# THUDM/CogView

Measured on AMD Instinct MI355X. Metric: train tokens/sec/node (seq1089, 4B GPT) at 1/2/4/8 MI355X; % MFMA roofline, higher is better.
Workload: dtype fp16

## Files before the change

### cogview_amd/_lib.py

```python
import ctypes as C
import os

_HERE = os.path.dirname(os.path.abspath(__file__))
LIB_PATH = os.environ.get("COGVIEW_HIP_LIB") or os.path.join(_HERE, "lib", "libcogview_hip.so")

F16, BF16, F32 = 0, 1, 2
EPI_BIAS, EPI_GELU, EPI_DGELU, EPI_DROPOUT, EPI_ABSMAX, EPI_ACCUM, EPI_COLSUM = 1, 2, 4, 8, 16, 32, 64
EPI_GELU_DAUX, EPI_MULAUX = 128, 256

_ERR = {1: "bad argument (shape / alignment / dtype)", 2: "kernel launch failure", 3: "unsupported combination"}


class CogviewHipError(RuntimeError):
    pass


class GemmDesc(C.Structure):
    _fields_ = [
        ("dtype", C.c_int), ("trans_a", C.c_int), ("trans_b", C.c_int),
        ("M", C.c_int), ("N", C.c_int), ("K", C.c_int),
        ("A", C.c_void_p), ("lda", C.c_int),
        ("B", C.c_void_p), ("ldb", C.c_int),
        ("C", C.c_void_p), ("ldc", C.c_int),
        ("out_f32", C.c_int), ("flags", C.c_int),
# ... 148 lines not shown


CONV_4X4_S2, CONV_1X1, CONVT_4X4_S2, CONV_3X3_S1 = 0, 1, 2, 3
CONV_FP32, CONV_BF16X3 = 0, 1

_vp, _i, _f, _u64, _i64, _sz = C.c_void_p, C.c_int, C.c_float, C.c_uint64, C.c_int64, C.c_size_t

SIGNATURES = {
    "cogv_version": (_i, []),
    "cogv_arch": (C.c_char_p, []),
    "cogv_gemm": (_i, [C.POINTER(GemmDesc), _vp]),
    "cogv_gemm_workspace_bytes": (_sz, [C.POINTER(GemmDesc)]),
    "cogv_gemm_pick_splitk": (_i, [_i, _i, _i]),
    "cogv_gemm_grouped": (_i, [C.POINTER(GemmDesc), _i, _vp]),
    "cogv_gemm_colsum_rows": (_i, [_i]),
    "cogv_colsum_finalize": (_i, [_i, _vp, _i, _i, _vp, _i, _vp]),
    "cogv_gemm_pick_splitk_tiles": (_i, [_i, _i]),
    "cogv_sandwich_ln_fwd": (_i, [_i, _vp, _vp, _vp, _vp, _vp, _vp, _vp, _vp, _vp, _i, _i, _f, _i, _vp]),
    "cogv_sandwich_ln_bwd": (_i, [_i, _vp, _vp, _vp, _vp, _vp, _vp, _vp, _vp, _vp, _vp, _i, _i, _i, _f, _u64, _u64,
                                  _vp, _sz, _i, _vp]),
    "cogv_sandwich_ln_bwd_marked": (_i, [_i, _vp, _vp, _vp, _vp, _vp, _vp, _vp, _vp, _vp, _vp, _i, _i, _i, _f, _vp, _sz, _i, _vp]),
    "cogv_ln_bwd_workspace_bytes": (_sz, [_i, _i]),
    "cogv_sandwich_ln_bwd_pair": (_i, [_i, _vp, _vp, _vp, _vp, _vp, _vp, _vp, _vp, _vp, _vp, _vp, _vp, _vp, _vp, _vp, _vp, _vp, _i, _i, _i, _f,
                                       _vp, _sz, _vp]),
    "cogv_ln_bwd_pair_workspace_bytes": (_sz, [_i, _i]),
    "cogv_ln_bwd_num_blocks": (_i, [_i]),
    "cogv_ln_bwd_plan": (_i, [_i, _i, _i, _f, _i, _i, C.POINTER(C.c_int)]),
    "cogv_ln_bwd_pair_plan": (_i, [_i, _i, _f, C.POINTER(C.c_int)]),
    "cogv_gemm_reserve_cus": (_i, [_i]),
    "cogv_gemm_plan": (_i, [C.POINTER(GemmDesc), _i, _i, C.POINTER(C.c_int)]),
    "cogv_attention_fwd": (_i, [C.POINTER(AttnDesc), _vp]),
    "cogv_attention_bwd": (_i, [C.POINTER(AttnDesc), _vp]),
    "cogv_attention_plan": (_i, [C.POINTER(AttnDesc), _i, C.POINTER(C.c_int)]),
    "cogv_gemv_ln": (_i, [C.POINTER(GemmDesc), C.POINTER(LnPrologue), _vp]),
    "cogv_gemv_attn": (_i, [C.POINTER(GemmDesc), _vp, _i, _i, _vp]),
    "cogv_attention_decode": (_i, [C.POINTER(AttnDecodeDesc), _vp]),
    "cogv_attention_decode_chunk": (_i, [C.POINTER(AttnDecodeChunkDesc), _vp]),
    "cogv_quantize_rows_e4m3": (_i, [_i, _vp, _i, _i, _i, _vp, _i, _vp, _vp]),
    "cogv_gemm_w8": (_i, [C.POINTER(GemmDesc), C.POINTER(W8Weight), _vp]),
    "cogv_gemv_ln_w8": (_i, [C.POINTER(GemmDesc), C.POINTER(LnPrologue), C.POINTER(W8Weight), _vp]),
    "cogv_gemv_attn_w8": (_i, [C.POINTER(GemmDesc), C.POINTER(W8Weight), _vp, _i, _i, _vp]),
    "cogv_gemv_plan": (_i, [_i, C.POINTER(GemmDesc), C.POINTER(W8Weight), _i, C.POINTER(C.c_int)]),
    "cogv_quantize_rows_mxfp4": (_i, [_i, _vp, _i, _i, _i, _vp, _i, _vp, _i, _vp]),
    "cogv_gemm_w4": (_i, [C.POINTER(GemmDesc), C.POINTER(W4Weight), _vp]),
    "cogv_gemv_ln_w4": (_i, [C.POINTER(GemmDesc), C.POINTER(LnPrologue), C.POINTER(W4Weight), _vp]),
    "cogv_gemv_attn_w4": (_i, [C.POINTER(GemmDesc), C.POINTER(W4Weight), _vp, _i, _i, _vp]),
    "cogv_gemv_w4_plan": (_i, [_i, C.POINTER(GemmDesc), C.POINTER(W4Weight), _i, C.POINTER(C.c_int)]),
    "cogv_gemm_rows": (_i, [C.POINTER(GemmDesc), _vp]),
    "cogv_gemm_rows_plan": (_i, [C.POINTER(GemmDesc), C.POINTER(C.c_int)]),
    "cogv_kv_quantize_e4m3": (_i, [_i, _vp, _i64, _i64, _i, _i, _i, _vp, _i64, _vp, _i64, _i, _i, _vp]),
    "cogv_attention_decode_kv8": (_i, [C.POINTER(AttnDecodeKv8Desc), _vp]),
    "cogv_attention_decode_workspace_bytes": (_sz, [_i, _i, _i]),
    "cogv_attention_keep_bits_bytes": (_sz, [_i, _i, _i, _i]),
    "cogv_sparse_slot_reduce": (_i, [_i, _vp, _vp, _vp, _vp, _vp, _i64, _i, _i64, _i, _i, _i, _i, _i, _i, _i, _vp]),
    "cogv_embedding_fwd": (_i, [_i, _vp, _vp, _i64, _i64, _vp, _vp, _vp, _i64, _vp, _vp, _i64, _i, _f, _u64, _u64, _i, _vp]),
    "cogv_embedding_bwd": (_i, [_i, _vp, _vp, _vp, _i64, _i64, _vp, _vp, _i64, _vp, _i64, _i, _f, _u64, _u64, _vp, _sz, _i, _vp]),
    "cogv_embedding_bwd_workspace_bytes": (_sz, [_i64, _i64]),
    "cogv_gelu_fwd": (_i, [_i, _vp, _vp, _sz, _vp]),
    "cogv_gelu_bwd": (_i, [_i, _vp, _vp, _vp, _sz, _vp]),
    "cogv_dropout": (_i, [_i, _vp, _vp, _sz, _f, _u64, _u64, _vp, _vp]),
    "cogv_add": (_i, [_i, _vp, _vp, _vp, _sz, _vp, _vp]),
    "cogv_add_stream": (_i, [_i, _vp, _vp, _vp, _sz, _vp, _vp]),
    "cogv_scale": (_i, [_i, _vp, _vp, _sz, _f, _vp]),
    "cogv_absmax": (_i, [_i, _vp, _sz, _vp, _vp]),
    "cogv_colsum": (_i, [_i, _vp, _i, _i, _i, _vp, _i, _vp, _sz, _vp]),
    "cogv_colsum_workspace_bytes": (_sz, [_i, _i]),
# ... 156 lines not shown
```

### cogview_amd/csrc/attention.hip

```cpp
#include "common.cuh"
#include "cogview_hip.h"

#include <type_traits>

namespace {

constexpr int HD = 64;
constexpr int NT = 256;
constexpr float MASKED = -10000.0f;
constexpr int TILE = 8192;
#ifndef COGV_ATTN_STAGES
#define COGV_ATTN_STAGES 2
#endif
constexpr int NSTG = COGV_ATTN_STAGES;
static_assert(NSTG == 2 || NSTG == 3, "ring of two or three stages");
constexpr int COLSUM_SMEM = (128 * 68 + 256) * 4;

constexpr int DMA_TILE = 2;
template <int SIZE_, int DMAS_, bool COLSUM_> struct RingStage {
  static constexpr int SIZE = SIZE_, DMAS = DMAS_, INDEX = NSTG * SIZE_;
  static constexpr int dynamic_lds(int index_slots) {
    return ((COLSUM_ && INDEX < COLSUM_SMEM) ? COLSUM_SMEM : INDEX) + ((index_slots * 4 + 15) / 16) * 16;
  }
};
struct FwdStage : RingStage<2 * TILE, 2 * DMA_TILE, false> { static constexpr int K = 0, V = TILE; };
constexpr int DQ_KW_PITCH = 256;
template <bool KB> struct DqStage : RingStage<2 * TILE + (KB ? 4 * DQ_KW_PITCH : 0), 2 * DMA_TILE + (KB ? 1 : 0), true> {
  static constexpr int K = 0, V = TILE, KW = 2 * TILE, KW_PITCH = DQ_KW_PITCH;
};
constexpr int DKDV_KW_PITCH = 272;
template <bool KB> struct DkdvStage : RingStage<2 * TILE + 512 + (KB ? 4 * DKDV_KW_PITCH : 256), 2 * DMA_TILE + 3, true> {
  static constexpr int Q = 0, DO = TILE, LSE = 2 * TILE, D = LSE + 256;
  static constexpr int RK = D + 256, KW = D + 256, KW_PITCH = DKDV_KW_PITCH;
};

struct AttnArgs {
  const void* q; const void* k; const void* v; void* o;
  const void* dout; void* dq; void* dk; void* dv;
  float* lse; float* dvec;
  float* colsum_ws;
  uint32_t* keepbits;
  const void* mask; long long mask_bs;
  const int* kv_index; long long kv_index_bs;
  long long kv_index_gs; int sp_w, sp_npiv; float sp_bias;
  long long q_bs, k_bs, v_bs, o_bs, do_bs, dq_bs, dk_bs, dv_bs;
  int q_rs, k_rs, v_rs, o_rs, do_rs, dq_rs, dk_rs, dv_rs;
  int B, H, s_q, s_k, sep_k;
  float scale;
  uint32_t thr16; float keep_scale; uint32_t rng_key;
};

struct BlockId { int bx, head, z; bool ok; };
__device__ __forceinline__ BlockId xcd_block_id(int nx, int H, int Z, bool heavy_last) {
  const int L = blockIdx.x, x = L & 7, j = L >> 3;
  const int ul = j / nx, k = j - ul * nx;
  const int u = ul * 8 + x;
  BlockId id;
  id.ok = u < H * Z;
  id.z = u / H; id.head = u - id.z * H;
  id.bx = heavy_last ? nx - 1 - k : k;
  return id;
}

typedef __attribute__((address_space(3))) void lds_void_t;
typedef __attribute__((address_space(1))) const void gbl_void_t;

template <int N> __device__ __forceinline__ void wait_vmcnt() { asm volatile("s_waitcnt vmcnt(%0)" ::"n"(N) : "memory"); }

__device__ __forceinline__ int aswz(int row) { return (((row >> 1) & 1) << 2) | ((row >> 2) & 3); }

template <typename T>
__device__ __forceinline__ void dma_tile(const T* base, long long rs, int row0, int nrows, char* lds, int wave, int lane,
                                         const int* lds_index = nullptr) {
#pragma unroll
  for (int i = 0; i < DMA_TILE; ++i) {
    const int piece = wave + 4 * i;
    const int row = piece * 8 + (lane >> 3);
    const int c = (lane & 7) ^ aswz(row);
    int gr = min(row0 + row, nrows - 1);
    if (lds_index) {
      const uint32_t a = (uint32_t)(uintptr_t)(lds_index + gr);
      asm volatile("ds_read_b32 %0, %1\n\ts_waitcnt lgkmcnt(0)" : "=v"(gr) : "v"(a) : "memory");
// ... 87 lines not shown
__device__ __forceinline__ bool keep_of(const u32x2& r, int i, uint32_t thr16) {
  return (i & 1) ? (r[i >> 1] >= (thr16 << 16)) : ((r[i >> 1] & 0xffffu) >= thr16);
}

template <typename T, int SB>
__device__ __forceinline__ void tr_frags_issue(uint32_t tile_addr, const uint32_t (&loff)[2], TrRaw (&r)[2][2]) {
#pragma unroll
  for (int d = 0; d < 2; ++d) { tr_issue<SB * 32>(tile_addr, loff[d], r[0][d]); tr_issue<SB * 32 + 16>(tile_addr, loff[d], r[1][d]); }
}

template <typename T, int SB>
__device__ __forceinline__ void tr_frags_sync(uint32_t tile_addr, const uint32_t (&loff)[2], TrRaw (&r)[2][2]) {
  constexpr int S0 = SB * 32, S1 = SB * 32 + 16;
  constexpr int XA = (((S0 >> 3) & 1) << 1) << 4, XB = ((((S0 + 8) >> 3) & 1) << 1) << 4;
  constexpr int XC = (((S1 >> 3) & 1) << 1) << 4, XD = ((((S1 + 8) >> 3) & 1) << 1) << 4;
  uint32_t a[2][4];
#pragma unroll
  for (int d = 0; d < 2; ++d) {
    a[d][0] = tile_addr + S0 * 128 + (loff[d] ^ XA);
    a[d][1] = tile_addr + (S0 + 8) * 128 + (loff[d] ^ XB);
    a[d][2] = tile_addr + S1 * 128 + (loff[d] ^ XC);
    a[d][3] = tile_addr + (S1 + 8) * 128 + (loff[d] ^ XD);
  }
  asm volatile(
      "ds_read_b64_tr_b16 %0, %8\n\tds_read_b64_tr_b16 %1, %9\n\tds_read_b64_tr_b16 %2, %10\n\tds_read_b64_tr_b16 %3, %11\n\t"
      "ds_read_b64_tr_b16 %4, %12\n\tds_read_b64_tr_b16 %5, %13\n\tds_read_b64_tr_b16 %6, %14\n\tds_read_b64_tr_b16 %7, %15\n\t"
      "s_waitcnt lgkmcnt(0)"
      : "=&v"(r[0][0].lo), "=&v"(r[0][0].hi), "=&v"(r[1][0].lo), "=&v"(r[1][0].hi),
        "=&v"(r[0][1].lo), "=&v"(r[0][1].hi), "=&v"(r[1][1].lo), "=&v"(r[1][1].hi)
      : "v"(a[0][0]), "v"(a[0][1]), "v"(a[0][2]), "v"(a[0][3]), "v"(a[1][0]), "v"(a[1][1]), "v"(a[1][2]), "v"(a[1][3])
      : "memory");
}

__device__ __forceinline__ void tile_colsum(const float (&vals)[2][16], float* lds, float* dst, int lane, int wave) {
  constexpr int PITCH = 68;
  const int fr = lane & 31, fg = lane >> 5;
  float* row = lds + (wave * 32 + fr) * PITCH;
#pragma unroll
  for (int d = 0; d < 2; ++d)
#pragma unroll
    for (int gq = 0; gq < 4; ++gq)
      *reinterpret_cast<f32x4*>(row + 32 * d + 8 * gq + 4 * fg) =
          f32x4{vals[d][4 * gq], vals[d][4 * gq + 1], vals[d][4 * gq + 2], vals[d][4 * gq + 3]};
  __syncthreads();
  const int col = threadIdx.x & 63, slice = threadIdx.x >> 6;
  float s0 = 0.f, s1 = 0.f;
#pragma unroll
  for (int r = 0; r < 32; r += 2) {
    s0 += lds[(slice * 32 + r) * PITCH + col];
    s1 += lds[(slice * 32 + r + 1) * PITCH + col];
  }
  float* red = lds + 128 * PITCH;
  red[slice * 64 + col] = s0 + s1;
  __syncthreads();
  if (threadIdx.x < 64) dst[threadIdx.x] = red[threadIdx.x] + red[64 + threadIdx.x] + red[128 + threadIdx.x] + red[192 + threadIdx.x];
  __syncthreads();
}

template <bool IDX> __device__ __forceinline__ int* stage_index_table(const AttnArgs& p, int b, int gblk, char* behind_ring) {
  if (!(IDX && p.kv_index)) return nullptr;
  int* lidx = reinterpret_cast<int*>(behind_ring);
  const int* gi = p.kv_index + (long long)b * p.kv_index_bs + (long long)gblk * p.kv_index_gs;
  for (int i = threadIdx.x; i < p.s_k; i += NT) lidx[i] = gi[i];
  __syncthreads();
  return lidx;
}
struct SlotAttrs { unsigned long long masked, pivot; };
__device__ __forceinline__ SlotAttrs slot_attrs(const int* lidx, int kb, int lane, const AttnArgs& p) {
  int raw;
  const uint32_t ia = (uint32_t)(uintptr_t)(lidx + min(kb * 64 + lane, p.s_k - 1));
  asm volatile("ds_read_b32 %0, %1\n\ts_waitcnt lgkmcnt(0)" : "=v"(raw) : "v"(ia) : "memory");
  SlotAttrs a;
  a.masked = __ballot(raw < 0); a.pivot = __ballot(kb * 64 + lane < p.sp_npiv);
  return a;
}
__device__ __forceinline__ void apply_slot_attrs(f32x16& s, const SlotAttrs& a, int sb, int fg, float masked_raw, float bias_raw) {
  const uint32_t fm = (uint32_t)(a.masked >> (32 * sb)) >> (4 * fg), pm = (uint32_t)(a.pivot >> (32 * sb)) >> (4 * fg);
#pragma unroll
  for (int e = 0; e < 16; ++e) {
    const int bit = elem_idx(e);
    float v = s[e];
    v = ((fm >> bit) & 1u) ? masked_raw : v;
    v += ((pm >> bit) & 1u) ? bias_raw : 0.f;
    s[e] = v;
  }
}
template <typename T> __device__ __forceinline__ void apply_mask_tensor(f32x16& s, float (&mk)[16], const AttnArgs& p, int b, int myq,
                                                                        int kfirst, int fg, float masked_raw) {
  const T* mrow = reinterpret_cast<const T*>(p.mask) + (long long)b * p.mask_bs + (long long)min(myq, p.s_q - 1) * p.s_k;
#pragma unroll
  for (int e = 0; e < 16; ++e) {
    const int key = kfirst + 4 * fg + elem_idx(e);
    mk[e] = HT<T>::to_f(mrow[min(key, p.s_k - 1)]);
    s[e] = fmaf(s[e], mk[e], masked_raw * (1.f - mk[e]));
  }
}
template <int NF> __device__ __forceinline__ void mask_edge(f32x16* s, int kfirst, int q0w, int myq, int off, int fg, const AttnArgs& p,
                                                            float masked_raw) {
  const bool all_visible = (kfirst + (32 * NF - 1) <= q0w + off) || (kfirst + (32 * NF - 1) < p.sep_k);
  if (!all_visible || kfirst + 32 * NF > p.s_k) {
#pragma unroll
    for (int sb = 0; sb < NF; ++sb) {
      const int base = kfirst + sb * 32 + 4 * fg;
      mask_frag(s[sb], myq + off - base, p.sep_k - base, p.s_k - base, masked_raw);
    }
  }
}

template <typename T, bool IDX, int DROP>
__global__ __launch_bounds__(NT, 2) void attn_fwd_kernel(const AttnArgs p) {
  const bool drop = DROP < 0 ? (p.thr16 != 0u) : (DROP != 0);
  extern __shared__ __attribute__((aligned(16))) char smem[];
  using L = FwdStage;
  const int lane = threadIdx.x & 63;
  const int wave = __builtin_amdgcn_readfirstlane(threadIdx.x >> 6);
  const int fr = lane & 31, fg = lane >> 5;
  const int nblk_x = (p.s_q + 127) >> 7;
  const BlockId bid = xcd_block_id(nblk_x, p.H, p.B, true);
  if (!bid.ok) return;
  const int b = bid.z, head = bid.head;
  const int q0 = bid.bx * 128, q0w = q0 + wave * 32;
  const bool spw = IDX && p.sp_w > 0;
  const int gblk = spw ? q0 / p.sp_w : 0;
  const int off = spw ? (p.s_k - p.sp_w - gblk * p.sp_w) : (p.s_k - p.s_q);
  const T* Q = reinterpret_cast<const T*>(p.q) + b * p.q_bs + head * HD;
  const T* K = reinterpret_cast<const T*>(p.k) + b * p.k_bs + head * HD;
  const T* V = reinterpret_cast<const T*>(p.v) + b * p.v_bs + head * HD;
  const int myq = q0w + fr;
  const bool wave_active = q0w < p.s_q;

  typename HT<T>::v8 qf[4];
#pragma unroll
  for (int t = 0; t < 4; ++t) qf[t] = load_frag_global<T>(Q + (long long)myq * p.q_rs + 16 * t + 8 * fg, myq < p.s_q);

  const int q_last = min(p.s_q, q0 + 128) - 1;
  const int kend_blk = min(p.s_k, max(q_last + off + 1, p.sep_k));
  const int nkb = (kend_blk + 63) >> 6;
  const int qw_last = min(p.s_q, q0w + 32) - 1;
  const int kend_w = wave_active ? min(p.s_k, max(qw_last + off + 1, p.sep_k)) : 0;

  f32x16 oacc[2];
#pragma unroll
  for (int d = 0; d < 2; ++d)
#pragma unroll
    for (int e = 0; e < 16; ++e) oacc[d][e] = 0.f;
  float m_run = -INFINITY, l_run = 0.f;
  const float sl2 = p.scale * 1.4426950408889634f;
  const float masked_raw = MASKED / p.scale;
  const long long arow = ((long long)b * p.H + head) * p.s_q + myq;
  const RowKey cb = row_key(p.rng_key, (unsigned long long)arow);
  const float kofs = drop ? __builtin_amdgcn_logf(p.keep_scale) : 0.f;
  const uint32_t loff[2] = {tr_lane_off(0, lane) ^ tr_lane_fix(lane), tr_lane_off(1, lane) ^ tr_lane_fix(lane)};
  const uint32_t smem_addr = (uint32_t)(uintptr_t)smem;

  int* const lidx = stage_index_table<IDX>(p, b, gblk, smem + L::INDEX);
  const float sp_bias_raw = spw ? p.sp_bias / p.scale : 0.f;
  auto issue = [&](int kb, int st) {
    dma_tile<T>(K, p.k_rs, kb * 64, p.s_k, smem + st * L::SIZE + L::K, wave, lane, lidx);
    dma_tile<T>(V, p.v_rs, kb * 64, p.s_k, smem + st * L::SIZE + L::V, wave, lane, lidx);
  };
  static_assert(L::DMAS == 2 * DMA_TILE, "issue(): K tile, V tile");
  uint32_t* const kwp = DROP == 2 ? p.keepbits + ((((long long)b * p.H + head) * ((p.s_k + 63) >> 6)) * 2 + fg) * p.s_q + min(myq, p.s_q - 1) : nullptr;
  if (nkb > 0) { issue(0, 0); if (NSTG > 2) issue(nkb > 1 ? 1 : 0, 1); }
  int st = 0;
  for (int kb = 0; kb < nkb; ++kb) {
    wait_vmcnt<(NSTG - 2) * L::DMAS>();
    __builtin_amdgcn_s_barrier();
    issue(min(kb + NSTG - 1, nkb - 1), st == 0 ? NSTG - 1 : st - 1);
    if (kb * 64 < kend_w) {
      const char* lk = smem + st * L::SIZE + L::K;
      const uint32_t lv = smem_addr + st * L::SIZE + L::V;
      f32x16 sacc[2];
#pragma unroll
      for (int sb = 0; sb < 2; ++sb) {
#pragma unroll
        for (int e = 0; e < 16; ++e) sacc[sb][e] = 0.f;
#pragma unroll
        for (int t = 0; t < 4; ++t)
          sacc[sb] = HT<T>::mfma32(nat_frag<T>(lk, sb * 32 + fr, 2 * t + fg), qf[t], sacc[sb]);
      }
      TrRaw vr[2][2];
      tr_frags_issue<T, 0>(lv, loff, vr);
      if (IDX && lidx) {
        const SlotAttrs sa = slot_attrs(lidx, kb, lane, p);
#pragma unroll
        for (int sb = 0; sb < 2; ++sb) apply_slot_attrs(sacc[sb], sa, sb, fg, masked_raw, sp_bias_raw);
      }
      const int kfirst = kb * 64;
      if (IDX && p.mask) {
        float mk[16];
#pragma unroll
        for (int sb = 0; sb < 2; ++sb) apply_mask_tensor<T>(sacc[sb], mk, p, b, myq, kfirst + sb * 32, fg, masked_raw);
      }
      mask_edge<2>(sacc, kfirst, q0w, myq, off, fg, p, masked_raw);
      float mb = sacc[0][0];
// ... 12 lines not shown
      if (!__all(mb <= m_run)) {
        const float m_new = fmaxf(m_run, mb);
        const float alpha = fast_exp2(m_run - m_new);
        m_run = m_new;
        l_run *= alpha;
#pragma unroll
        for (int d = 0; d < 2; ++d)
#pragma unroll
          for (int e = 0; e < 16; ++e) oacc[d][e] *= alpha;
      }
      float ls = 0.f;
#pragma unroll
      for (int sb = 0; sb < 2; ++sb)
#pragma unroll
        for (int e = 0; e < 16; ++e) { const float pv = fast_exp2(fmaf(sacc[sb][e], sl2, kofs - m_run)); sacc[sb][e] = pv; ls += pv; }
      l_run += ls;
      if (drop) {
        uint32_t kw = 0u;
#pragma unroll
        for (int sb = 0; sb < 2; ++sb)
#pragma unroll
          for (int gq = 0; gq < 4; ++gq) {
            const u32x2 r = attn_bits_at(cb, (uint32_t)((kb * 64 + sb * 32 + 8 * gq + 4 * fg) >> 2));
#pragma unroll
            for (int i = 0; i < 4; ++i) {
              const bool kp = keep_of(r, i, p.thr16);
              sacc[sb][4 * gq + i] = kp ? sacc[sb][4 * gq + i] : 0.f;
              if (DROP == 2) {
                const unsigned long long cm = __ballot(kp);
                asm("v_addc_co_u32_e64 %0, vcc, %0, %0, %1" : "+v"(kw) : "s"(cm) : "vcc");
              }
            }
          }
        if (DROP == 2 && myq < p.s_q) kwp[(long long)kb * 2 * p.s_q] = kw;
      }
      TrRaw vr2[2][2];
      tr_wait(vr[0][0], vr[0][1]); tr_wait(vr[1][0], vr[1][1]);
      tr_frags_issue<T, 1>(lv, loff, vr2);
#pragma unroll
      for (int t = 0; t < 2; ++t) {
        float pe[8];
#pragma unroll
        for (int e = 0; e < 8; ++e) pe[e] = sacc[0][8 * t + e];
        const typename HT<T>::v8 pb = cvt8<T>(pe);
#pragma unroll
        for (int d = 0; d < 2; ++d) oacc[d] = HT<T>::mfma32(tr_pack<T>(vr[t][d]), pb, oacc[d]);
      }
      tr_wait(vr2[0][0], vr2[0][1]); tr_wait(vr2[1][0], vr2[1][1]);
#pragma unroll
      for (int t = 0; t < 2; ++t) {
        float pe[8];
#pragma unroll
        for (int e = 0; e < 8; ++e) pe[e] = sacc[1][8 * t + e];
        const typename HT<T>::v8 pb = cvt8<T>(pe);
#pragma unroll
        for (int d = 0; d < 2; ++d) oacc[d] = HT<T>::mfma32(tr_pack<T>(vr2[t][d]), pb, oacc[d]);
      }
    }
    st = (st == NSTG - 1) ? 0 : st + 1;
  }
  wait_vmcnt<0>();
  if (wave_active && myq < p.s_q) {
    const float l_tot = l_run + __shfl_xor(l_run, 32, 64);
    const float inv = (drop ? p.keep_scale : 1.0f) / l_tot;
    if (fg == 0 && p.lse) p.lse[((long long)b * p.H + head) * p.s_q + myq] = (m_run + __builtin_amdgcn_logf(l_tot) - kofs) * 0.6931471805599453f;
    T* O = reinterpret_cast<T*>(p.o) + b * p.o_bs + (long long)myq * p.o_rs + head * HD;
#pragma unroll
    for (int d = 0; d < 2; ++d)
#pragma unroll
      for (int gq = 0; gq < 4; ++gq) {
        u32x2 w;
        w[0] = pack2<T>(oacc[d][4 * gq] * inv, oacc[d][4 * gq + 1] * inv);
        w[1] = pack2<T>(oacc[d][4 * gq + 2] * inv, oacc[d][4 * gq + 3] * inv);
        *reinterpret_cast<u32x2*>(O + d * 32 + 8 * gq + 4 * fg) = w;
      }
  }
}

template <typename T, bool IDX, int DROP>
__global__ __launch_bounds__(NT, 2) void attn_bwd_dq_kernel(const AttnArgs p) {
  const bool drop = DROP < 0 ? (p.thr16 != 0u) : (DROP != 0);
  extern __shared__ __attribute__((aligned(16))) char smem[];
  constexpr bool KB = DROP == 2;
  using L = DqStage<KB>;
  const int lane = threadIdx.x & 63;
  const int wave = __builtin_amdgcn_readfirstlane(threadIdx.x >> 6);
  const int fr = lane & 31, fg = lane >> 5;
  const int nblk_x = (p.s_q + 127) >> 7;
  const BlockId bid = xcd_block_id(nblk_x, p.H, p.B, true);
  if (!bid.ok) return;
  const int b = bid.z, head = bid.head;
  const int q0 = bid.bx * 128, q0w = q0 + wave * 32;
  const bool spw = IDX && p.sp_w > 0;
  const int gblk = spw ? q0 / p.sp_w : 0;
  const int off = spw ? (p.s_k - p.sp_w - gblk * p.sp_w) : (p.s_k - p.s_q);
  const T* Q = reinterpret_cast<const T*>(p.q) + b * p.q_bs + head * HD;
  const T* K = reinterpret_cast<const T*>(p.k) + b * p.k_bs + head * HD;
  const T* V = reinterpret_cast<const T*>(p.v) + b * p.v_bs + head * HD;
  const T* DO = reinterpret_cast<const T*>(p.dout) + b * p.do_bs + head * HD;
  const int myq = q0w + fr;
  const bool qvalid = myq < p.s_q;
  const bool wave_active = q0w < p.s_q;

  typename HT<T>::v8 qf[4], dof[4];
#pragma unroll
  for (int t = 0; t < 4; ++t) {
    qf[t] = load_frag_global<T>(Q + (long long)myq * p.q_rs + 16 * t + 8 * fg, qvalid);
    dof[t] = load_frag_global<T>(DO + (long long)myq * p.do_rs + 16 * t + 8 * fg, qvalid);
  }
  const long long arow = ((long long)b * p.H + head) * p.s_q + myq;
  const RowKey cb = row_key(p.rng_key, (unsigned long long)arow);
  const float kscale = drop ? p.keep_scale : 1.0f;
  const float lse2 = qvalid ? p.lse[arow] * 1.4426950408889634f : 0.f;
  float dv = 0.f;
  {
    const T* Op = reinterpret_cast<const T*>(p.o) + b * p.o_bs + head * HD;
#pragma unroll
    for (int t = 0; t < 4; ++t) {
      const typename HT<T>::v8 of = load_frag_global<T>(Op + (long long)myq * p.o_rs + 16 * t + 8 * fg, qvalid);
#pragma unroll
      for (int e = 0; e < 8; ++e) dv = fmaf((float)dof[t][e], (float)of[e], dv);
    }
    dv += __shfl_xor(dv, 32, 64);
    if (qvalid && fg == 0) {
      p.dvec[arow] = -dv;
      if (!KB) reinterpret_cast<uint32_t*>(p.dvec)[(long long)p.B * p.H * p.s_q + arow] = cb.rk;
      else p.dvec[(long long)p.B * p.H * p.s_q + arow] = -lse2;
    }
  }
  const float sl2 = p.scale * 1.4426950408889634f;
  const float masked_raw = MASKED / p.scale;

  const int q_last = min(p.s_q, q0 + 128) - 1;
  const int kend_blk = min(p.s_k, max(q_last + off + 1, p.sep_k));
  const int nkb = (kend_blk + 63) >> 6;
  const int qw_last = min(p.s_q, q0w + 32) - 1;
  const int kend_w = wave_active ? min(p.s_k, max(qw_last + off + 1, p.sep_k)) : 0;

  f32x16 dqacc[2];
#pragma unroll
  for (int d = 0; d < 2; ++d)
#pragma unroll
    for (int e = 0; e < 16; ++e) dqacc[d][e] = 0.f;
  const uint32_t loff[2] = {tr_lane_off(0, lane) ^ tr_lane_fix(lane), tr_lane_off(1, lane) ^ tr_lane_fix(lane)};
  const uint32_t smem_addr = (uint32_t)(uintptr_t)smem;

  int* const lidx = stage_index_table<IDX>(p, b, gblk, smem + L::INDEX);
  const float sp_bias_raw = spw ? p.sp_bias / p.scale : 0.f;
  const uint32_t* KWQ = KB ? p.keepbits + ((long long)b * p.H + head) * ((p.s_k + 63) >> 6) * 2 * p.s_q + (long long)fg * p.s_q + min(myq, p.s_q - 1)
                           : nullptr;
  auto issue = [&](int kb, int st) {
    dma_tile<T>(K, p.k_rs, kb * 64, p.s_k, smem + st * L::SIZE + L::K, wave, lane, lidx);
    dma_tile<T>(V, p.v_rs, kb * 64, p.s_k, smem + st * L::SIZE + L::V, wave, lane, lidx);
    if (KB) __builtin_amdgcn_global_load_lds((gbl_void_t*)(KWQ + (long long)kb * 2 * p.s_q),
                                             (lds_void_t*)(smem + st * L::SIZE + L::KW + wave * L::KW_PITCH), 4, 0, 0);
  };
  static_assert(L::DMAS == 2 * DMA_TILE + (KB ? 1 : 0), "issue(): K tile, V tile, KB: the wave's keep words");
  if (nkb > 0) { issue(0, 0); if (NSTG > 2) issue(nkb > 1 ? 1 : 0, 1); }
  int st = 0;
  for (int kb = 0; kb < nkb; ++kb) {
    wait_vmcnt<(NSTG - 2) * L::DMAS>();
    __builtin_amdgcn_s_barrier();
    issue(min(kb + NSTG - 1, nkb - 1), st == 0 ? NSTG - 1 : st - 1);
    if (kb * 64 < kend_w) {
      const char* lk = smem + st * L::SIZE + L::K; const char* lv = smem + st * L::SIZE + L::V;
      const uint32_t lkt = smem_addr + st * L::SIZE + L::K;
      uint32_t kwv = 0u;
      if (KB) {
        const uint32_t ka = smem_addr + st * L::SIZE + L::KW + wave * L::KW_PITCH + lane * 4;
        asm volatile("ds_read_b32 %0, %1\n\ts_waitcnt lgkmcnt(0)" : "=v"(kwv) : "v"(ka) : "memory");
      }
      SlotAttrs sa = {0ull, 0ull};
      if (spw) sa = slot_attrs(lidx, kb, lane, p);
      auto half = [&](auto SBc) {
        constexpr int sb = decltype(SBc)::value;
        f32x16 sacc, pacc;
#pragma unroll
        for (int e = 0; e < 16; ++e) { sacc[e] = 0.f; pacc[e] = 0.f; }
#pragma unroll
        for (int t = 0; t < 4; ++t) {
          sacc = HT<T>::mfma32(nat_frag<T>(lk, sb * 32 + fr, 2 * t + fg), qf[t], sacc);
          pacc = HT<T>::mfma32(nat_frag<T>(lv, sb * 32 + fr, 2 * t + fg), dof[t], pacc);
// ... 32 lines not shown
        tr_wait(kr[0][0], kr[0][1]); tr_wait(kr[1][0], kr[1][1]);
#pragma unroll
        for (int t = 0; t < 2; ++t) {
          const typename HT<T>::v8 dsb = cvt8<T>(ds + 8 * t);
#pragma unroll
          for (int d = 0; d < 2; ++d) dqacc[d] = HT<T>::mfma32(tr_pack<T>(kr[t][d]), dsb, dqacc[d]);
        }
      };
      half(std::integral_constant<int, 0>{});
      half(std::integral_constant<int, 1>{});
    }
    st = (st == NSTG - 1) ? 0 : st + 1;
  }
  wait_vmcnt<0>();
  float rq[2][16];
  {
    T* DQ = reinterpret_cast<T*>(p.dq) + b * p.dq_bs + (long long)myq * p.dq_rs + head * HD;
#pragma unroll
    for (int d = 0; d < 2; ++d)
#pragma unroll
      for (int gq = 0; gq < 4; ++gq) {
        u32x2 w;
        w[0] = pack2<T>(dqacc[d][4 * gq] * p.scale, dqacc[d][4 * gq + 1] * p.scale);
        w[1] = pack2<T>(dqacc[d][4 * gq + 2] * p.scale, dqacc[d][4 * gq + 3] * p.scale);
        if (qvalid) *reinterpret_cast<u32x2*>(DQ + d * 32 + 8 * gq + 4 * fg) = w;
#pragma unroll
        for (int i = 0; i < 4; ++i)
          rq[d][4 * gq + i] = qvalid ? bits_to_f<T>((uint16_t)(w[i >> 1] >> (16 * (i & 1)))) : 0.f;
      }
  }
  if (p.colsum_ws) {
    __syncthreads();
    float* dst = p.colsum_ws + ((size_t)b * nblk_x + bid.bx) * (size_t)(3 * p.H * HD) + head * HD;
    tile_colsum(rq, reinterpret_cast<float*>(smem), dst, lane, wave);
  }
}

#if defined(COGV_ATTN_TS)
__device__ unsigned long long g_attn_ts[1024 * 8];
#define ATS(k_) do { const unsigned long long t_ = __builtin_readcyclecounter(); ats[k_] += t_ - ats_last; ats_last = t_; } while (0)
#else
#define ATS(k_) do { } while (0)
#endif
template <typename T, bool IDX, int DROP>
__global__ __launch_bounds__(NT, 2) void attn_bwd_dkdv_kernel(const AttnArgs p) {
  const bool drop = DROP < 0 ? (p.thr16 != 0u) : (DROP != 0);
  extern __shared__ __attribute__((aligned(16))) char smem[];
  constexpr bool KB = DROP == 2;
  using L = DkdvStage<KB>;
#if defined(COGV_ATTN_TS)
  unsigned long long ats[8] = {0, 0, 0, 0, 0, 0, 0, 0};
  const unsigned long long ats_begin = __builtin_readcyclecounter();
  unsigned long long ats_last = ats_begin;
#endif
  const int lane = threadIdx.x & 63;
  const int wave = __builtin_amdgcn_readfirstlane(threadIdx.x >> 6);
  const int fr = lane & 31, fg = lane >> 5;
  const bool spw = IDX && p.sp_w > 0;
  const int nblk = spw ? p.s_q / p.sp_w : 1;
  const int nblk_x = (p.s_k + 127) >> 7;
  const BlockId bid = xcd_block_id(nblk_x, p.H, p.B * nblk, false);
  if (!bid.ok) return;
  const int zb = bid.z, head = bid.head;
  const int b = spw ? zb / nblk : zb, gblk = spw ? zb - b * nblk : 0;
  const int k0 = bid.bx * 128, k0w = k0 + wave * 32;
  const int off = spw ? (p.s_k - p.sp_w - gblk * p.sp_w) : (p.s_k - p.s_q);
  const int qlo = gblk * p.sp_w, qhi = spw ? qlo + p.sp_w : p.s_q;
  const T* Q = reinterpret_cast<const T*>(p.q) + b * p.q_bs + head * HD;
// ... 254 lines not shown
#pragma unroll
  for (int which = 0; which < 2; ++which) {
    const T* src = (which ? dvs : dks) + (long long)b * G * n_slots * slot_row + c * 8;
    float acc[8];
#pragma unroll
    for (int i = 0; i < 8; ++i) acc[i] = 0.f;
    auto add = [&](int g, int slot) {
      const u32x4 raw = *reinterpret_cast<const u32x4*>(src + ((long long)g * n_slots + slot) * slot_row);
#pragma unroll
      for (int i = 0; i < 8; ++i) acc[i] += bits_to_f<T>((uint16_t)(raw[i >> 1] >> (16 * (i & 1))));
    };
    const int gend = min(G - 1, g0 + times - 1);
    for (int g = g0; g <= gend; ++g) add(g, n_piv + r - (g - times + 1) * w);
    if (pj >= 0)
      for (int g = g0 + times; g < G; ++g) add(g, pj);
    u32x4 o;
#pragma unroll
    for (int i = 0; i < 4; ++i) o[i] = pack2<T>(acc[2 * i], acc[2 * i + 1]);
    T* dst = which ? dv + b * dv_bs + (long long)r * dv_rs + c * 8 : dk + b * dk_bs + (long long)r * dk_rs + c * 8;
    *reinterpret_cast<u32x4*>(dst) = o;
  }
}

inline bool aligned16(const void* p) { return ((uintptr_t)p & 15) == 0; }

enum AttnForm { ATTN_DENSE = 0, ATTN_DENSE_DROP = 1, ATTN_DENSE_BITS = 2, ATTN_FLEXIBLE = 3 };

struct AttnPlan {
  int form;
  AttnArgs a;
  unsigned grid_q, grid_k;
  int lds_q, lds_k;
  int planes;
};

int index_args(const cogv_attn_desc* d, AttnArgs& a) {
  if (d->kv_index) {
    if (a.s_k > 4096) return COGV_ERR_UNSUPPORTED;
    a.kv_index = d->kv_index; a.kv_index_bs = d->kv_index_bs;
    if (d->sparse_window > 0) {
      if ((d->sparse_window % 128) || (a.s_q % d->sparse_window) || d->sparse_pivots < 0 || d->sparse_pivots > a.s_k ||
          a.s_k < d->sparse_window || a.sep_k != 0) return COGV_ERR_ARG;
      a.kv_index_gs = d->kv_index_gs; a.sp_w = d->sparse_window; a.sp_npiv = d->sparse_pivots; a.sp_bias = d->sparse_pivot_bias;
    }
  } else if (d->sparse_window > 0) {
    return COGV_ERR_ARG;
  }
  return COGV_OK;
}

int attn_plan(const cogv_attn_desc* d, bool backward, AttnPlan& pl) {
  AttnArgs& a = pl.a;
  if (!d) return COGV_ERR_ARG;
  if (d->dtype != COGV_F16 && d->dtype != COGV_BF16) return COGV_ERR_UNSUPPORTED;
  if (d->head_dim != HD) return COGV_ERR_UNSUPPORTED;
  if (d->B <= 0 || d->H <= 0 || d->s_q <= 0 || d->s_k <= 0) return COGV_ERR_ARG;
  if (d->s_k < d->s_q && !(d->kv_index && d->sparse_window > 0)) return COGV_ERR_ARG;
  if (!(d->dropout_p >= 0.f && d->dropout_p < 1.f)) return COGV_ERR_ARG;
  a.q = d->q; a.k = d->k; a.v = d->v; a.o = d->o; a.dout = d->dout; a.dq = d->dq; a.dk = d->dk; a.dv = d->dv;
  a.lse = d->lse; a.dvec = d->dvec; a.colsum_ws = nullptr; a.kv_index = nullptr; a.kv_index_bs = 0;
  a.keepbits = nullptr; a.mask = nullptr; a.mask_bs = 0;
  if (d->mask) {
    if (((uintptr_t)d->mask & 1) || d->kv_index || d->keep_bits) return COGV_ERR_ARG;
    a.mask = d->mask; a.mask_bs = d->mask_bs;
  }
  a.kv_index_gs = 0; a.sp_w = 0; a.sp_npiv = 0; a.sp_bias = 0.f;
  a.q_bs = d->q_bs; a.k_bs = d->k_bs; a.v_bs = d->v_bs; a.o_bs = d->o_bs; a.do_bs = d->do_bs;
// ... 15 lines not shown
    if (!aligned16(a.q) || !aligned16(a.k) || !aligned16(a.v) || !aligned16(a.o)) return COGV_ERR_ARG;
    if ((a.q_rs | a.k_rs | a.v_rs | a.o_rs) & 7) return COGV_ERR_ARG;
    if ((a.q_bs | a.k_bs | a.v_bs | a.o_bs) & 7) return COGV_ERR_ARG;
    if ((rc = index_args(d, a))) return rc;
  } else {
    if (!a.dout || !a.dq || !a.dk || !a.dv || !a.lse || !a.dvec) return COGV_ERR_ARG;
    if (d->kv_index && d->sparse_window <= 0) return COGV_ERR_UNSUPPORTED;
    if ((rc = index_args(d, a))) return rc;
    if (a.sp_w > 0 && d->colsum_partial) return COGV_ERR_UNSUPPORTED;
    if (d->colsum_partial) {
      if (d->s_q != d->s_k || ((uintptr_t)d->colsum_partial & 15)) return COGV_ERR_ARG;
      a.colsum_ws = d->colsum_partial;
    }
    if (!aligned16(a.q) || !aligned16(a.k) || !aligned16(a.v) || !aligned16(a.o) || !aligned16(a.dout) ||
        !aligned16(a.dq) || !aligned16(a.dk) || !aligned16(a.dv)) return COGV_ERR_ARG;
    if ((a.q_rs | a.k_rs | a.v_rs | a.o_rs | a.do_rs | a.dq_rs | a.dk_rs | a.dv_rs) & 7) return COGV_ERR_ARG;
    if ((a.q_bs | a.k_bs | a.v_bs | a.o_bs | a.do_bs | a.dq_bs | a.dk_bs | a.dv_bs) & 7) return COGV_ERR_ARG;
  }
  const int slots = a.kv_index ? a.s_k : 0;
  pl.planes = a.sp_w > 0 && backward ? a.B * (a.s_q / a.sp_w) : a.B;
  pl.grid_q = 8u * (unsigned)((a.H * a.B + 7) / 8) * (unsigned)((a.s_q + 127) / 128);
  pl.grid_k = backward ? 8u * (unsigned)((a.H * pl.planes + 7) / 8) * (unsigned)((a.s_k + 127) / 128) : 0u;
  pl.lds_q = backward ? DqStage<false>::dynamic_lds(slots) : FwdStage::dynamic_lds(slots);
  pl.lds_k = backward ? DkdvStage<false>::dynamic_lds(0) : 0;
  if (pl.lds_q > 160 * 1024) return COGV_ERR_UNSUPPORTED;
  const bool drop = a.thr16 != 0u;
  pl.form = (a.kv_index || a.mask) ? ATTN_FLEXIBLE : drop ? ATTN_DENSE_DROP : ATTN_DENSE;
  if (d->keep_bits && drop && !a.kv_index) {
    if ((uintptr_t)d->keep_bits & 3) return COGV_ERR_ARG;
    a.keepbits = reinterpret_cast<uint32_t*>(d->keep_bits);
    pl.form = ATTN_DENSE_BITS;
    if (backward) { pl.lds_q = DqStage<true>::dynamic_lds(0); pl.lds_k = DkdvStage<true>::dynamic_lds(0); }
  }
  return COGV_OK;
}

template <void (*KERNEL)(const AttnArgs)>
void attn_launch(unsigned grid, int lds, hipStream_t st, const AttnArgs& a) {
  static int raised = 0;
  if (lds > raised) {
    (void)hipFuncSetAttribute(reinterpret_cast<const void*>(KERNEL), hipFuncAttributeMaxDynamicSharedMemorySize, lds);
    raised = lds;
  }
  hipLaunchKernelGGL(KERNEL, dim3(grid), dim3(NT), lds, st, a);
}
template <typename T, bool IDX, int DROP>
void attn_launch_form(const AttnPlan& pl, bool backward, hipStream_t st) {
  if (!backward) return attn_launch<attn_fwd_kernel<T, IDX, DROP>>(pl.grid_q, pl.lds_q, st, pl.a);
  attn_launch<attn_bwd_dq_kernel<T, IDX, DROP>>(pl.grid_q, pl.lds_q, st, pl.a);
  attn_launch<attn_bwd_dkdv_kernel<T, IDX, DROP>>(pl.grid_k, pl.lds_k, st, pl.a);
}
template <typename T>
void attn_launch_dtype(const AttnPlan& pl, bool backward, hipStream_t st) {
  switch (pl.form) {
    case ATTN_DENSE: return attn_launch_form<T, false, 0>(pl, backward, st);
    case ATTN_DENSE_DROP: return attn_launch_form<T, false, 1>(pl, backward, st);
    case ATTN_DENSE_BITS: return attn_launch_form<T, false, 2>(pl, backward, st);
    default: return attn_launch_form<T, true, -1>(pl, backward, st);
  }
}
int attn_run(const cogv_attn_desc* d, bool backward, void* stream) {
  AttnPlan pl;
  const int rc = attn_plan(d, backward, pl);
  if (rc) return rc;
  hipStream_t st = reinterpret_cast<hipStream_t>(stream);
  if (d->dtype == COGV_F16) attn_launch_dtype<f16_t>(pl, backward, st);
  else attn_launch_dtype<bf16_t>(pl, backward, st);
  return cogv_check_launch();
}

}

extern "C" int cogv_attention_fwd(const cogv_attn_desc* d, void* stream) { return attn_run(d, false, stream); }
extern "C" int cogv_attention_bwd(const cogv_attn_desc* d, void* stream) { return attn_run(d, true, stream); }

extern "C" int cogv_attention_plan(const cogv_attn_desc* d, int backward, int out[8]) {
  AttnPlan pl;
  const int rc = attn_plan(d, backward != 0, pl);
  if (rc || !out) return rc ? rc : COGV_ERR_ARG;
  out[0] = pl.form; out[1] = NT; out[2] = (int)pl.grid_q; out[3] = pl.lds_q; out[4] = (int)pl.grid_k; out[5] = pl.lds_k;
  out[6] = pl.planes; out[7] = pl.a.sep_k;
  return COGV_OK;
}

extern "C" size_t cogv_attention_keep_bits_bytes(int B, int H, int s_q, int s_k) {
  if (B <= 0 || H <= 0 || s_q <= 0 || s_k <= 0) return 0;
  return (size_t)B * H * ((size_t)(s_k + 63) / 64) * 2 * (size_t)s_q * sizeof(uint32_t);
}

extern "C" int cogv_sparse_slot_reduce(int dtype, const void* dk_slots, const void* dv_slots, const int* pivot_inv,
                                       void* dk, void* dv, long long dk_bs, int dk_rs, long long dv_bs, int dv_rs,
                                       int B, int s, int H, int window, int times, int n_pivots, void* stream) {
  if (dtype != COGV_F16 && dtype != COGV_BF16) return COGV_ERR_UNSUPPORTED;
  if (!dk_slots || !dv_slots || !pivot_inv || !dk || !dv) return COGV_ERR_ARG;
  if (B <= 0 || s <= 0 || H <= 0 || window <= 0 || times <= 0 || n_pivots < 0 || (s % window)) return COGV_ERR_ARG;
  if (!aligned16(dk_slots) || !aligned16(dv_slots) || !aligned16(dk) || !aligned16(dv)) return COGV_ERR_ARG;
  if ((dk_bs | dv_bs | dk_rs | dv_rs) & 7) return COGV_ERR_ARG;
  const int C8 = H * HD / 8;
  const long long total = (long long)B * s * C8;
  const unsigned blocks = (unsigned)((total + 255) / 256);
  hipStream_t st = reinterpret_cast<hipStream_t>(stream);
  if (dtype == COGV_F16)
    hipLaunchKernelGGL((sparse_slot_reduce_kernel<f16_t>), dim3(blocks), dim3(256), 0, st, (const f16_t*)dk_slots,
                       (const f16_t*)dv_slots, pivot_inv, (f16_t*)dk, (f16_t*)dv, dk_bs, dk_rs, dv_bs, dv_rs, B, s, C8,
                       window, times, n_pivots);
  else
    hipLaunchKernelGGL((sparse_slot_reduce_kernel<bf16_t>), dim3(blocks), dim3(256), 0, st, (const bf16_t*)dk_slots,
                       (const bf16_t*)dv_slots, pivot_inv, (bf16_t*)dk, (bf16_t*)dv, dk_bs, dk_rs, dv_bs, dv_rs, B, s, C8,
                       window, times, n_pivots);
  return cogv_check_launch();
}

#if defined(COGV_ATTN_TS)
extern "C" int cogv_debug_attn_ts(unsigned long long* host_out, int reset) {
// ... 13 lines not shown
```

### include/cogview_hip.h

```cpp
#ifndef COGVIEW_HIP_H
#define COGVIEW_HIP_H

#include <stddef.h>
#include <stdint.h>

#ifdef __cplusplus
extern "C" {
#endif

#define COGV_F16 0
#define COGV_BF16 1
#define COGV_F32 2

int cogv_version(void);
const char* cogv_arch(void);

#define COGV_EPI_BIAS 1
#define COGV_EPI_GELU 2
#define COGV_EPI_DGELU 4
#define COGV_EPI_DROPOUT 8
#define COGV_EPI_ABSMAX 16
#define COGV_EPI_ACCUM 32
#define COGV_EPI_COLSUM 64

// ... 82 lines not shown
int cogv_sandwich_ln_bwd_marked(int dtype, const void* dy, const void* x, const void* gamma, const float* mean,
                                const float* rstd, const void* add_in, void* dx, void* dgamma, void* dbeta, void* colsum,
                                int accumulate_param_grads, int rows, int h, float dropout_p, void* workspace,
                                size_t workspace_bytes, int stream_mode, void* stream);
int cogv_sandwich_ln_bwd_pair(int dtype, const void* dc, const void* y, const void* gamma2, const float* mean2,
                              const float* rstd2, const void* dout, void* dy, void* dgamma2, void* dbeta2,
                              const void* ao, const void* gamma3, const float* mean3, const float* rstd3, void* d_ao,
                              void* dgamma3, void* dbeta3, void* colsum, int accumulate_param_grads, int rows, int h,
                              float dropout_p, void* workspace, size_t workspace_bytes, void* stream);
size_t cogv_ln_bwd_pair_workspace_bytes(int rows, int h);
size_t cogv_ln_bwd_workspace_bytes(int rows, int h);
int cogv_ln_bwd_num_blocks(int rows);
int cogv_ln_bwd_plan(int stream_mode, int rows, int h, float dropout_p, int marked, int has_add_in, int out[5]);
int cogv_ln_bwd_pair_plan(int rows, int h, float dropout_p, int out[5]);

typedef struct cogv_attn_desc {
  int dtype; int B, H, s_q, s_k, head_dim; int sep;
  float scale;
  float dropout_p; uint64_t seed; uint64_t stream_id;
  const void* q; const void* k; const void* v; void* o;
  const void* dout; void* dq; void* dk; void* dv;
  float* lse; float* dvec;
  long long q_bs, k_bs, v_bs, o_bs, do_bs, dq_bs, dk_bs, dv_bs;
  int q_rs, k_rs, v_rs, o_rs, do_rs, dq_rs, dk_rs, dv_rs;
  float* colsum_partial;
  const int* kv_index; long long kv_index_bs;
  long long kv_index_gs; int sparse_window, sparse_pivots; float sparse_pivot_bias;
  void* keep_bits;
  const void* mask; long long mask_bs;
} cogv_attn_desc;
int cogv_attention_fwd(const cogv_attn_desc* d, void* stream);
int cogv_attention_bwd(const cogv_attn_desc* d, void* stream);
int cogv_attention_plan(const cogv_attn_desc* d, int backward, int out[8]);
size_t cogv_attention_keep_bits_bytes(int B, int H, int s_q, int s_k);
typedef struct cogv_attn_decode_desc {
  int dtype; int B, H, capacity, head_dim;
  float scale;
  const void* qkv; long long qkv_bs;
  void* cache; long long cache_bs; int cache_rs;
  void* out; long long out_bs;
  const long long* pos;
  void* workspace; size_t workspace_bytes;
  int skip_combine;
  const int* first;
} cogv_attn_decode_desc;
size_t cogv_attention_decode_workspace_bytes(int B, int H, int capacity);
int cogv_attention_decode(const cogv_attn_decode_desc* d, void* stream);
typedef struct cogv_attn_decode_chunk_desc {
  int dtype; int B, H, capacity, head_dim;
  int m;
  float scale;
  const void* qkv; long long qkv_rs;
  void* cache; long long cache_bs; int cache_rs;
  void* out; long long out_rs;
  const long long* pos;
  void* workspace; size_t workspace_bytes;
  int skip_combine;
  const int* first;
} cogv_attn_decode_chunk_desc;
int cogv_attention_decode_chunk(const cogv_attn_decode_chunk_desc* d, void* stream);
int cogv_kv_quantize_e4m3(int dtype, const void* kv, long long kv_bs, long long kv_rs, int B, int n, int H, void* q, long long q_bs,
                          float* scale, long long scale_bs, int capacity, int slot0, void* stream);
typedef struct cogv_attn_decode_kv8_desc {
  int dtype; int B, H, capacity, head_dim;
  float scale;
  const void* qkv; long long qkv_bs;
// ... 156 lines not shown
```

Before: 43080.

## Shift query tiling so the partial tile sits first in causal attention

When s_q is not a multiple of 128, the dense causal forward and backward-dq kernels now start their query blocks shifted backwards by a multiple of 32 rows. The partial block becomes the first one, which sees the fewest keys, so the last block is full and the number of padded key-block steps falls. The dq colsum epilogue splits its per-wave partial sums across adjacent block slots, and a small regroup kernel merges them afterwards. This adds a kernel launch and index bookkeeping in exchange for less wasted causal work. An env var can restore front alignment.

```diff
diff --git a/cogview_amd/_lib.py b/cogview_amd/_lib.py
--- a/cogview_amd/_lib.py
+++ b/cogview_amd/_lib.py
@@ -204,6 +204,7 @@
     "cogv_attention_fwd": (_i, [C.POINTER(AttnDesc), _vp]),
     "cogv_attention_bwd": (_i, [C.POINTER(AttnDesc), _vp]),
     "cogv_attention_plan": (_i, [C.POINTER(AttnDesc), _i, C.POINTER(C.c_int)]),
+    "cogv_attention_query_cut": (_i, [_i, _i, _i, C.POINTER(C.c_int)]),
     "cogv_gemv_ln": (_i, [C.POINTER(GemmDesc), C.POINTER(LnPrologue), _vp]),
     "cogv_gemv_attn": (_i, [C.POINTER(GemmDesc), _vp, _i, _i, _vp]),
     "cogv_attention_decode": (_i, [C.POINTER(AttnDecodeDesc), _vp]),
diff --git a/cogview_amd/csrc/attention.hip b/cogview_amd/csrc/attention.hip
--- a/cogview_amd/csrc/attention.hip
+++ b/cogview_amd/csrc/attention.hip
@@ -1,6 +1,9 @@
 #include "common.cuh"
 #include "cogview_hip.h"
 
+#include <algorithm>
+#include <cstdlib>
+#include <cstring>
 #include <type_traits>
 
 namespace {
@@ -48,6 +51,7 @@
   int B, H, s_q, s_k, sep_k;
   float scale;
   uint32_t thr16; float keep_scale; uint32_t rng_key;
+  int q_shift;
 };
 
 struct BlockId { int bx, head, z; bool ok; };
@@ -201,7 +205,8 @@
       : "memory");
 }
 
-__device__ __forceinline__ void tile_colsum(const float (&vals)[2][16], float* lds, float* dst, int lane, int wave) {
+__device__ __forceinline__ void tile_colsum(const float (&vals)[2][16], float* lds, float* dst, int lane, int wave, int lead = 0,
+                                            float* dst_lead = nullptr, size_t lead_pitch = 0) {
   constexpr int PITCH = 68;
   const int fr = lane & 31, fg = lane >> 5;
   float* row = lds + (wave * 32 + fr) * PITCH;
@@ -222,7 +227,17 @@
   float* red = lds + 128 * PITCH;
   red[slice * 64 + col] = s0 + s1;
   __syncthreads();
-  if (threadIdx.x < 64) dst[threadIdx.x] = red[threadIdx.x] + red[64 + threadIdx.x] + red[128 + threadIdx.x] + red[192 + threadIdx.x];
+  if (threadIdx.x < 64) {
+    if (lead == 0) {
+      dst[threadIdx.x] = red[threadIdx.x] + red[64 + threadIdx.x] + red[128 + threadIdx.x] + red[192 + threadIdx.x];
+    } else {
+      float s = red[lead * 64 + threadIdx.x];
+      for (int i = lead + 1; i < 4; ++i) s += red[i * 64 + threadIdx.x];
+      dst[threadIdx.x] = s;
+      if (dst_lead)
+        for (int i = 0; i < lead; ++i) dst_lead[i * lead_pitch + threadIdx.x] = red[i * 64 + threadIdx.x];
+    }
+  }
   __syncthreads();
 }
 
@@ -288,7 +303,7 @@
   const BlockId bid = xcd_block_id(nblk_x, p.H, p.B, true);
   if (!bid.ok) return;
   const int b = bid.z, head = bid.head;
-  const int q0 = bid.bx * 128, q0w = q0 + wave * 32;
+  const int q0 = bid.bx * 128 - (IDX ? 0 : p.q_shift), q0w = q0 + wave * 32;
   const bool spw = IDX && p.sp_w > 0;
   const int gblk = spw ? q0 / p.sp_w : 0;
   const int off = spw ? (p.s_k - p.sp_w - gblk * p.sp_w) : (p.s_k - p.s_q);
@@ -296,11 +311,12 @@
   const T* K = reinterpret_cast<const T*>(p.k) + b * p.k_bs + head * HD;
   const T* V = reinterpret_cast<const T*>(p.v) + b * p.v_bs + head * HD;
   const int myq = q0w + fr;
-  const bool wave_active = q0w < p.s_q;
+  const bool qvalid = (IDX || myq >= 0) && myq < p.s_q;
+  const bool wave_active = (IDX || q0w >= 0) && q0w < p.s_q;
 
   typename HT<T>::v8 qf[4];
 #pragma unroll
-  for (int t = 0; t < 4; ++t) qf[t] = load_frag_global<T>(Q + (long long)myq * p.q_rs + 16 * t + 8 * fg, myq < p.s_q);
+  for (int t = 0; t < 4; ++t) qf[t] = load_frag_global<T>(Q + (long long)myq * p.q_rs + 16 * t + 8 * fg, qvalid);
 
   const int q_last = min(p.s_q, q0 + 128) - 1;
   const int kend_blk = min(p.s_k, max(q_last + off + 1, p.sep_k));
@@ -329,7 +345,7 @@
     dma_tile<T>(V, p.v_rs, kb * 64, p.s_k, smem + st * L::SIZE + L::V, wave, lane, lidx);
   };
   static_assert(L::DMAS == 2 * DMA_TILE, "issue(): K tile, V tile");
-  uint32_t* const kwp = DROP == 2 ? p.keepbits + ((((long long)b * p.H + head) * ((p.s_k + 63) >> 6)) * 2 + fg) * p.s_q + min(myq, p.s_q - 1) : nullptr;
+  uint32_t* const kwp = DROP == 2 ? p.keepbits + ((((long long)b * p.H + head) * ((p.s_k + 63) >> 6)) * 2 + fg) * p.s_q + min(max(myq, 0), p.s_q - 1) : nullptr;
   if (nkb > 0) { issue(0, 0); if (NSTG > 2) issue(nkb > 1 ? 1 : 0, 1); }
   int st = 0;
   for (int kb = 0; kb < nkb; ++kb) {
@@ -408,7 +424,7 @@
               }
             }
           }
-        if (DROP == 2 && myq < p.s_q) kwp[(long long)kb * 2 * p.s_q] = kw;
+        if (DROP == 2 && qvalid) kwp[(long long)kb * 2 * p.s_q] = kw;
       }
       TrRaw vr2[2][2];
       tr_wait(vr[0][0], vr[0][1]); tr_wait(vr[1][0], vr[1][1]);
@@ -436,7 +452,7 @@
     st = (st == NSTG - 1) ? 0 : st + 1;
   }
   wait_vmcnt<0>();
-  if (wave_active && myq < p.s_q) {
+  if (wave_active && qvalid) {
     const float l_tot = l_run + __shfl_xor(l_run, 32, 64);
     const float inv = (drop ? p.keep_scale : 1.0f) / l_tot;
     if (fg == 0 && p.lse) p.lse[((long long)b * p.H + head) * p.s_q + myq] = (m_run + __builtin_amdgcn_logf(l_tot) - kofs) * 0.6931471805599453f;
@@ -466,7 +482,7 @@
   const BlockId bid = xcd_block_id(nblk_x, p.H, p.B, true);
   if (!bid.ok) return;
   const int b = bid.z, head = bid.head;
-  const int q0 = bid.bx * 128, q0w = q0 + wave * 32;
+  const int q0 = bid.bx * 128 - (IDX ? 0 : p.q_shift), q0w = q0 + wave * 32;
   const bool spw = IDX && p.sp_w > 0;
   const int gblk = spw ? q0 / p.sp_w : 0;
   const int off = spw ? (p.s_k - p.sp_w - gblk * p.sp_w) : (p.s_k - p.s_q);
@@ -475,8 +491,8 @@
   const T* V = reinterpret_cast<const T*>(p.v) + b * p.v_bs + head * HD;
   const T* DO = reinterpret_cast<const T*>(p.dout) + b * p.do_bs + head * HD;
   const int myq = q0w + fr;
-  const bool qvalid = myq < p.s_q;
-  const bool wave_active = q0w < p.s_q;
+  const bool qvalid = (IDX || myq >= 0) && myq < p.s_q;
+  const bool wave_active = (IDX || q0w >= 0) && q0w < p.s_q;
 
   typename HT<T>::v8 qf[4], dof[4];
 #pragma unroll
@@ -523,7 +539,7 @@
 
   int* const lidx = stage_index_table<IDX>(p, b, gblk, smem + L::INDEX);
   const float sp_bias_raw = spw ? p.sp_bias / p.scale : 0.f;
-  const uint32_t* KWQ = KB ? p.keepbits + ((long long)b * p.H + head) * ((p.s_k + 63) >> 6) * 2 * p.s_q + (long long)fg * p.s_q + min(myq, p.s_q - 1)
+  const uint32_t* KWQ = KB ? p.keepbits + ((long long)b * p.H + head) * ((p.s_k + 63) >> 6) * 2 * p.s_q + (long long)fg * p.s_q + min(max(myq, 0), p.s_q - 1)
                            : nullptr;
   auto issue = [&](int kb, int st) {
     dma_tile<T>(K, p.k_rs, kb * 64, p.s_k, smem + st * L::SIZE + L::K, wave, lane, lidx);
@@ -622,8 +638,22 @@
   if (p.colsum_ws) {
     __syncthreads();
     float* dst = p.colsum_ws + ((size_t)b * nblk_x + bid.bx) * (size_t)(3 * p.H * HD) + head * HD;
-    tile_colsum(rq, reinterpret_cast<float*>(smem), dst, lane, wave);
-  }
+    const int lead = IDX ? 0 : p.q_shift >> 5;
+    tile_colsum(rq, reinterpret_cast<float*>(smem), dst, lane, wave, lead,
+                bid.bx > 0 ? dst - (size_t)(3 * p.H * HD) + (size_t)p.H * HD : nullptr, (size_t)p.H * HD);
+  }
+}
+
+__global__ __launch_bounds__(256) void attn_colsum_regroup_kernel(float* ws, int nblk, int HC, long long total, int lead) {
+  const long long tid = (long long)blockIdx.x * 256 + threadIdx.x;
+  if (tid >= total) return;
+  const int c = (int)(tid % HC);
+  const long long r = tid / HC;
+  const long long b = r / (nblk - 1), j = r - b * (nblk - 1);
+  float* q = ws + (b * nblk + j) * 3 * HC + c;
+  float s = q[0] + q[HC];
+  if (lead == 2) s += q[2 * HC];
+  q[0] = s;
 }
 
 #if defined(COGV_ATTN_TS)
@@ -944,7 +974,25 @@
   unsigned grid_q, grid_k;
   int lds_q, lds_k;
   int planes;
+  bool regroup;
 };
+
+int query_shift(int s_q) {
+  const int rem = s_q % 128;
+  return rem ? 128 - 32 * ((rem + 31) / 32) : 0;
+}
+int query_cut_steps(int s_q, int s_k, int shift) {
+  int steps = 0;
+  for (int bx = 0; bx < (s_q + 127) / 128; ++bx) {
+    const int q_last = std::min(s_q, bx * 128 - shift + 128) - 1;
+    steps += (std::min(s_k, q_last + (s_k - s_q) + 1) + 63) >> 6;
+  }
+  return steps;
+}
+bool query_cut_front() {
+  const char* e = getenv("COGV_ATTN_QALIGN");
+  return e && !strcmp(e, "front");
+}
 
 int index_args(const cogv_attn_desc* d, AttnArgs& a) {
   if (d->kv_index) {
@@ -1026,6 +1074,9 @@
     pl.form = ATTN_DENSE_BITS;
     if (backward) { pl.lds_q = DqStage<true>::dynamic_lds(0); pl.lds_k = DkdvStage<true>::dynamic_lds(0); }
   }
+  a.q_shift = (pl.form == ATTN_FLEXIBLE || query_cut_front()) ? 0 : query_shift(a.s_q);
+  if (backward && a.colsum_ws && a.q_shift > 64) a.q_shift = 0;
+  pl.regroup = backward && a.colsum_ws && a.q_shift > 0 && a.s_q > 128;
   return COGV_OK;
 }
 
@@ -1042,6 +1093,12 @@
 void attn_launch_form(const AttnPlan& pl, bool backward, hipStream_t st) {
   if (!backward) return attn_launch<attn_fwd_kernel<T, IDX, DROP>>(pl.grid_q, pl.lds_q, st, pl.a);
   attn_launch<attn_bwd_dq_kernel<T, IDX, DROP>>(pl.grid_q, pl.lds_q, st, pl.a);
+  if (pl.regroup) {
+    const int nblk = (pl.a.s_q + 127) / 128, HC = pl.a.H * HD;
+    const long long total = (long long)pl.a.B * (nblk - 1) * HC;
+    hipLaunchKernelGGL(attn_colsum_regroup_kernel, dim3((unsigned)((total + 255) / 256)), dim3(256), 0, st, pl.a.colsum_ws, nblk, HC,
+                       total, pl.a.q_shift >> 5);
+  }
   attn_launch<attn_bwd_dkdv_kernel<T, IDX, DROP>>(pl.grid_k, pl.lds_k, st, pl.a);
 }
 template <typename T>
@@ -1074,6 +1131,14 @@
   if (rc || !out) return rc ? rc : COGV_ERR_ARG;
   out[0] = pl.form; out[1] = NT; out[2] = (int)pl.grid_q; out[3] = pl.lds_q; out[4] = (int)pl.grid_k; out[5] = pl.lds_k;
   out[6] = pl.planes; out[7] = pl.a.sep_k;
+  return COGV_OK;
+}
+
+extern "C" int cogv_attention_query_cut(int s_q, int s_k, int align, int out[2]) {
+  if (s_q <= 0 || s_k < s_q || align < -1 || align > 1 || !out) return COGV_ERR_ARG;
+  const bool front = align < 0 ? query_cut_front() : align == 0;
+  out[0] = front ? 0 : query_shift(s_q);
+  out[1] = query_cut_steps(s_q, s_k, out[0]);
   return COGV_OK;
 }
 
diff --git a/include/cogview_hip.h b/include/cogview_hip.h
--- a/include/cogview_hip.h
+++ b/include/cogview_hip.h
@@ -138,6 +138,7 @@
 int cogv_attention_fwd(const cogv_attn_desc* d, void* stream);
 int cogv_attention_bwd(const cogv_attn_desc* d, void* stream);
 int cogv_attention_plan(const cogv_attn_desc* d, int backward, int out[8]);
+int cogv_attention_query_cut(int s_q, int s_k, int align, int out[2]);
 size_t cogv_attention_keep_bits_bytes(int B, int H, int s_q, int s_k);
 typedef struct cogv_attn_decode_desc {
   int dtype; int B, H, capacity, head_dim;
```

After: 43190 (median of 6 runs). About the same (+0.3%).
